# jmatta1/MCMCpp

Hardware: AMD Instinct MI355X
Metric: walker-steps/sec + acceptance rate, 16384 walkers x 32 dims, 1/2/4/8 GPU (higher is better)
Workload: dtype f64

## Files before the change

### mcmcpp_amd/csrc/mcmcpp_hip.hip

```cpp
#include <hip/hip_runtime.h>

#include <chrono>
#include <cmath>
#include <cstdarg>
#include <cstdio>
#include <cstdlib>
#include <cstring>
#include <map>
#include <mutex>
#include <new>
#include <string>
#include <thread>
#include <vector>

#include "../../include/mcmcpp_hip.h"
#define MCMCPP_DEFINE_REDUCE_KERNEL
#include "launch_table.hpp"
#include "sampler_host.hpp"
#include "split_exchange.hpp"

using namespace mcmcpp;

namespace
{
thread_local std::string g_create_error;

void parallel_memcpy(char* dst, const char* src, size_t bytes)
{
    const size_t kMinPiece = 512u << 10;
    int pieces = (int)(bytes / kMinPiece);
    if (pieces > 4) pieces = 4;
    if (pieces < 2)
    {
        std::memcpy(dst, src, bytes);
        return;
    }
    const size_t piece = ((bytes / (size_t)pieces) + 63) & ~(size_t)63;
    std::thread helpers[3];
    for (int k = 1; k < pieces; ++k)
    {
        const size_t off = piece * (size_t)k;
        const size_t len = (k == pieces - 1) ? bytes - off : piece;
        helpers[k - 1] = std::thread([=]() { std::memcpy(dst + off, src + off, len); });
    }
    std::memcpy(dst, src, piece);
    for (int k = 1; k < pieces; ++k) helpers[k - 1].join();
}

struct RegisteredCalc
{
    const void* f64;
    const void* f32;
    int params_len;
};
std::mutex g_registry_mutex;
std::map<int, RegisteredCalc> g_registry;

bool registered_calc(int calc_id, RegisteredCalc* out)
{
    std::lock_guard<std::mutex> lock(g_registry_mutex);
    std::map<int, RegisteredCalc>::const_iterator it = g_registry.find(calc_id);
    if (it == g_registry.end()) return false;
    if (out) *out = it->second;
    return true;
}

template <class T>
const LaunchTable<T>* table_for(int calc_id);
template <>
const LaunchTable<double>* table_for<double>(int calc_id)
{
    switch (calc_id)
    {
    case MCMCPP_HIP_CALC_ISO_GAUSSIAN: return launch_table_f64_iso();
    case MCMCPP_HIP_CALC_DENSE_GAUSSIAN: return launch_table_f64_dense();
    case MCMCPP_HIP_CALC_ROSENBROCK: return launch_table_f64_rosenbrock();
    case MCMCPP_HIP_CALC_SKEWED_GAUSSIAN_2D: return launch_table_f64_skewed();
    default:
    {
        RegisteredCalc r;
// ... 47 lines not shown
}
void launch_accepted_reduce(const uint32_t* partials, int partial_slots, int partial_waves, int count,
                            const StepCtl* ctl_after, const RunInfo* run, hipStream_t stream, int chains)
{
    hipLaunchKernelGGL(accepted_reduce_kernel, dim3((unsigned)count, (unsigned)(chains > 1 ? chains : 1)), dim3(256), 0, stream, partials, partial_slots,
                       partial_waves, count, ctl_after, run);
}
}

namespace
{
struct PinnedScratch
{
    alignas(64) StepCtl ctl;
    alignas(64) RunInfo run[4];
    alignas(64) StepCtl chain_ctl[kMaxChains];
    alignas(64) RunInfo chain_run[4][kMaxChains];
};
static_assert(sizeof(StepCtl) <= 64 && sizeof(RunInfo) <= 64, "a control or run record is uploaded as one 64-byte line");

int check_config(const mcmcpp_hip_config* c, std::string& err);

template <class T>
class Sampler final : public SamplerHost<T>
{
    MCMCPP_SAMPLER_HOST_NAMES;
    using Host::exchange_us_per_step, Host::xchg_bytes_per_step, Host::xchg_rollbacks, Host::xchg_cap_slots;

public:
    Sampler() {}
    ~Sampler() override
    {
        quiesce();
    }

    int init(const mcmcpp_hip_config& c)
    {
        cfg = c;
        knobs = Knobs::from_environment();
        set_shape(c);
        table = table_for<T>(c.calc_id);
        if (!table) return fail(MCMCPP_HIP_E_ARG, "calc_id %d has no kernels for this element type", c.calc_id);
        if (table->abi != kLaunchTableAbi || table->elem_size != sizeof(T))
            return fail(MCMCPP_HIP_E_ARG, "calc_id %d: the plug-in was built against other headers (table abi %08x)", c.calc_id, table->abi);

        const int lpw_log = ilog2(lpw), epl_shift = ilog2(epl / Vec16<T>::N);
        if (epl_shift >= kMaxEplShift || !table->half_step[lpw_log][epl_shift])
            return fail(MCMCPP_HIP_E_UNSUPPORTED, "no kernel for D=%d with this calculator (LPW=%d EPL=%d)", D, lpw, epl);
        calc_fn = table->calc[lpw_log][epl_shift];

        if (int rc = resolve_shard(c)) return rc;
        hipDeviceProp_t prop;
        if (int rc = open_device(c, &prop)) return rc;
        if (int rc = xchg.open(this, c)) return rc;
        K = c.num_chains > 1 ? c.num_chains : 1;
        if (K > kMaxChains) return fail(MCMCPP_HIP_E_ARG, "num_chains %d exceeds %d", K, kMaxChains);
        if (K > 1 && (shard_count != n || shard_begin != 0 || c.comm_world >= 1 || c.device_positions))
            return fail(MCMCPP_HIP_E_ARG, "num_chains > 1: whole ensembles on one device only (no shards, communicator or caller-owned positions)");
        if (int rc = open_stream(c)) return rc;

        StepShape s = {};
        s.W = W, s.D = D, s.n = n, s.lpw = lpw, s.elem_size = (int)sizeof(T), s.calc_id = c.calc_id;
        s.shard_begin = shard_begin, s.shard_count = shard_count, s.chains = K, s.comm_world = c.comm_world;
        s.num_cus = prop.multiProcessorCount;
        s.graph_steps = c.graph_steps;
        s.can_capture = own_stream || !(stream == nullptr || stream == hipStreamLegacy);
// ... 157 lines not shown
        if (!pos || !logp) return fail(MCMCPP_HIP_E_ARG, "set_state: null pointer");
        HIP_TRY(hipSetDevice(device));
        HIP_TRY(hipMemcpyAsync(d_pos, pos, sizeof(T) * (size_t)W * D * K, hipMemcpyHostToDevice, stream));
        for (int k = 0; k < K; ++k)
        {
            HIP_TRY(hipMemcpyAsync(logp_of(k), (const T*)logp + (size_t)k * W, sizeof(T) * (size_t)W, hipMemcpyHostToDevice, stream));
            HIP_TRY(hipMemsetAsync(nacc_of(k), 0, sizeof(uint32_t) * (size_t)W, stream));
        }
        HIP_TRY(hipMemsetAsync(d_diag, 0, sizeof(Diag), stream));
        half_steps = 0;
        steps_since_reset = 0;
        records_valid = false;
        int rc = write_ctl(half_steps, 0);
        if (rc) return rc;
        HIP_TRY(hipStreamSynchronize(stream));
        have_state = true;
        return MCMCPP_HIP_OK;
    }

    int run_mover(int64_t n_saved, int32_t interval, void* chain_out, uint32_t* accepted_per_step, bool to_device) override
    {
        return xchg.active() ? run_split(n_saved, interval, chain_out, accepted_per_step) : run_whole(n_saved, interval, chain_out, accepted_per_step, to_device);
    }
    int run_chains() const override { return K; }
    RunFacts run_facts() const override
    {
        RunFacts f = {};
        f.mover = Mover::Stretch;
        f.communicator = xchg.active();
        f.sharded = shard_count != n;
        f.half_done = (half_steps & 1) != 0;
        return f;
    }
    void state_abandoned() override { records_valid = false; }

    int begin_run(size_t acc_entries, const RunInfo* split_record)
    {
        if (acc_entries) HIP_TRY(hipMemsetAsync(d_acc, 0, sizeof(uint32_t) * acc_entries, stream));
        run_touched = true;
        if (int rc = write_ctl(half_steps, 0)) return rc;
        records_valid = false;
        run_info_idle = false;
        if (split_record) HIP_TRY(hipMemcpyAsync(d_run, split_record, sizeof(RunInfo), hipMemcpyHostToDevice, stream));
        if (full_fn)
        {
            for (int k = 0; k < K; ++k)
                hipLaunchKernelGGL(mark_rows_moved_kernel, dim3((unsigned)((W + 255) / 256)), dim3(256), 0, stream, nacc_of(k), W, kRowMovedBit);
            HIP_TRY(hipGetLastError());
        }
        enq_step = half_steps >> 1;
        run_step = 0;
        args_red = make_args(0);
        args_blk = make_args(1);
        return MCMCPP_HIP_OK;
    }

    using TimePoint = std::chrono::steady_clock::time_point;
    int finish_run(int64_t total, double gpu_ms, bool records_left, uint32_t* accepted_per_step, TimePoint tp1, TimePoint tp2)
    {
        last_ms = gpu_ms;
        last_launches = full_fn ? total : 2 * total;
        half_steps += 2 * (uint64_t)total;
        steps_since_reset += (uint64_t)total;
        records_valid = records_left;
        records_step = half_steps >> 1;
        records_partner2 = full_fn != nullptr;
        if (accepted_per_step) HIP_TRY(hipMemcpy(accepted_per_step, d_acc, sizeof(uint32_t) * (size_t)total * K, hipMemcpyDeviceToHost));
        host_enqueue_ms = std::chrono::duration<double, std::milli>(tp2 - tp1).count();
        return MCMCPP_HIP_OK;
    }

    int hand_out_staged(char* chain_out, const ChainPlan& cp, size_t step_bytes, StoredRange staged, int buf)
    {
        if (staged.to == staged.from) return MCMCPP_HIP_OK;
        HIP_TRY(hipEventSynchronize(ev_copied[buf]));
        for (int k = 0; k < K; ++k)
        {
            const SubchunkCopy c = subchunk_copy(step_bytes, cp.sub_saved, cp.n_saved, staged.from, staged.to - staged.from, k);
            std::memcpy(chain_out + c.dst, (const char*)h_stage[buf] + c.src, c.bytes);
        }
        publish_stored(staged.to);
        return MCMCPP_HIP_OK;
    }

    int run_whole(int64_t n_saved, int32_t interval, void* chain_out, uint32_t* accepted_per_step, bool to_device)
    {
        const int64_t total = n_saved * (int64_t)interval;

        const size_t step_bytes = sizeof(T) * (size_t)W * D;
        const ChainRequest want = {step_bytes, K, n_saved, interval, chain_out != nullptr, accepted_per_step != nullptr, full_fn != nullptr,
                                   chain_subchunk_bytes, plan.graph_steps, knobs.trickle, knobs.pinned_direct, to_device};
        void* direct_stage = pinned_question_matters(want) ? device_view_of_pinned(chain_out, step_bytes * (size_t)n_saved * K) : nullptr;
        const ChainPlan cp = plan_chain(want, direct_stage != nullptr);
        int rc = ensure_run_buffers(cp.acc_entries, cp.half_bytes, cp.ring_bytes, cp.need_host_ring);
        if (rc) return rc;
        if ((rc = begin_run(cp.acc_entries, nullptr))) return rc;
        if ((rc = ensure_graphs())) return rc;

        const TimePoint tp1 = std::chrono::steady_clock::now();
        double launch_ms = 0.0;
        if (cp.mode == ChainMode::Trickle)
            rc = run_trickle(n_saved, interval, (char*)chain_out, accepted_per_step != nullptr, step_bytes, cp, &launch_ms, (char*)direct_stage);
        else if (cp.mode == ChainMode::Device)
            rc = run_into_device_chain(n_saved, interval, (char*)chain_out, accepted_per_step != nullptr, step_bytes, cp, &launch_ms);
        StoredRange pending = {0, 0};
        int pending_buf = 0;
        for (int64_t c = 0; c < cp.n_sub && rc == MCMCPP_HIP_OK; ++c)
        {
            const int buf = (int)(c & 1);
            const StoredRange sub = cp.subchunk(c);
            for (int k = 0; k < K; ++k)
            {
                RunInfo* ri = K > 1 ? &h_pinned->chain_run[c % 4][k] : &h_pinned->run[c % 4];
                *ri = run_info_of_run(chain_out ? (char*)d_chain[buf].get() + subchunk_chain_offset(step_bytes, cp.sub_saved, k) : nullptr,
                                      accepted_per_step ? d_acc + (size_t)k * (size_t)total : nullptr, interval, step_bytes);
                ri->chain_slot_base = -sub.from;
                HIP_TRY(hipMemcpyAsync(run_of(k), ri, sizeof(RunInfo), hipMemcpyHostToDevice, stream));
            }
            HIP_TRY(hipEventRecord(ev_t0[c & 3], stream));
            rc = enqueue_steps((sub.to - sub.from) * interval);
            if (rc) break;
            HIP_TRY(hipEventRecord(ev_t1[c & 3], stream));
            if (c >= 3)
            {
                float ms = 0.f;
                HIP_TRY(hipEventSynchronize(ev_t1[(c - 3) & 3]));
                HIP_TRY(hipEventElapsedTime(&ms, ev_t0[(c - 3) & 3], ev_t1[(c - 3) & 3]));
                launch_ms += ms;
            }
            if (chain_out)
            {
                HIP_TRY(hipMemcpyAsync(h_stage[buf], d_chain[buf], subchunk_half_used(step_bytes, cp.sub_saved, sub.to - sub.from, K), hipMemcpyDeviceToHost, stream));
                HIP_TRY(hipEventRecord(ev_copied[buf], stream));
                if ((rc = hand_out_staged((char*)chain_out, cp, step_bytes, pending, pending_buf))) return rc;
                pending = sub;
// ... 172 lines not shown
    int enqueue_chunk(ChunkWindow& win, int64_t now)
    {
        const int e = win.event_slot(win.next_chunk);
        HIP_TRY(hipEventRecord(ev_t0[e], stream));
        if (const int rc = enqueue_steps(now)) return rc;
        HIP_TRY(hipEventRecord(ev_t1[e], stream));
        win.enqueued(now);
        return MCMCPP_HIP_OK;
    }
    int wait_for_oldest_chunk(const ChunkWindow& win, double* launch_ms)
    {
        const int e = win.event_slot(win.oldest);
        float ms = 0.f;
        HIP_TRY(hipEventSynchronize(ev_t1[e]));
        HIP_TRY(hipEventElapsedTime(&ms, ev_t0[e], ev_t1[e]));
        *launch_ms += ms;
        return MCMCPP_HIP_OK;
    }

    int run_trickle(int64_t n_saved, int32_t interval, char* chain_out, bool want_accepted, size_t step_bytes, const ChainPlan& cp, double* launch_ms,
                    char* direct_stage)
    {
        const int64_t total = n_saved * (int64_t)interval;
        const size_t ring_bytes = step_bytes * (size_t)cp.ring, out_bytes = step_bytes * (size_t)n_saved;
        for (int k = 0; k < K; ++k)
        {
            RunInfo* ri = &h_pinned->chain_run[0][k];
            *ri = run_info_of_run((char*)d_ring + ring_bytes * (size_t)k, want_accepted ? d_acc + (size_t)k * (size_t)total : nullptr, interval, step_bytes);
            ri->stage = cp.direct ? (void*)(direct_stage + out_bytes * (size_t)k) : (void*)((char*)h_ring + ring_bytes * (size_t)k);
            ri->slot_mask = cp.ring - 1;
            ri->slice_bytes = cp.slice_bytes;
            HIP_TRY(hipMemcpyAsync(run_of(k), ri, sizeof(RunInfo), hipMemcpyHostToDevice, stream));
        }

        TrickleWindow win(n_saved, interval, cp);
        auto copy_out = [&](StoredRange r, bool quick) {
            if (cp.direct) return;
            for (int64_t s = r.from; s < r.to; ++s)
                for (int k = 0; k < K; ++k)
                {
                    char* dst = chain_out + out_bytes * (size_t)k + step_bytes * (size_t)s;
                    const char* src = (char*)h_ring + ring_bytes * (size_t)k + step_bytes * (size_t)win.ring_slot(s);
                    if (quick)
                        parallel_memcpy(dst, src, step_bytes);
                    else
                        std::memcpy(dst, src, step_bytes);
                }
        };
        auto process_oldest = [&]() -> int {
            if (const int rc = wait_for_oldest_chunk(win, launch_ms)) return rc;
            copy_out(win.process_oldest(), win.all_enqueued());
            publish_stored(win.copied);
            return MCMCPP_HIP_OK;
        };
        while (!win.all_enqueued())
        {
            const int64_t now = win.next_length();
            while (win.must_process_oldest_before(now))
            {
                const int rc = process_oldest();
                if (rc) return rc;
            }
            if (const int rc = enqueue_chunk(win, now)) return rc;
        }
        for (int k = 0; k < K; ++k)
        {
            const size_t off = ring_bytes * (size_t)k + step_bytes * (size_t)win.ring_slot(n_saved - 1);
            char* dst = cp.direct ? chain_out + out_bytes * (size_t)k + step_bytes * (size_t)(n_saved - 1) : (char*)h_ring + off;
            HIP_TRY(hipMemcpyAsync(dst, (char*)d_ring + off, step_bytes, hipMemcpyDeviceToHost, stream));
        }
        while (win.in_flight())
        {
            const int rc = process_oldest();
            if (rc) return rc;
        }
        HIP_TRY(hipStreamSynchronize(stream));
        copy_out(win.tail(), true);
        publish_stored(win.copied);
        return MCMCPP_HIP_OK;
    }

    int run_into_device_chain(int64_t n_saved, int32_t interval, char* device_chain, bool want_accepted, size_t step_bytes, const ChainPlan& cp, double* launch_ms)
    {
        const int64_t total = n_saved * (int64_t)interval;
        for (int k = 0; k < K; ++k)
        {
            RunInfo* ri = &h_pinned->chain_run[0][k];
            *ri = run_info_of_run(device_chain + device_chain_offset(step_bytes, n_saved, k), want_accepted ? d_acc + (size_t)k * (size_t)total : nullptr, interval, step_bytes);
            HIP_TRY(hipMemcpyAsync(run_of(k), ri, sizeof(RunInfo), hipMemcpyHostToDevice, stream));
        }
        DeviceWindow win(n_saved, interval, cp);
        auto process_oldest = [&]() -> int {
            if (const int rc = wait_for_oldest_chunk(win, launch_ms)) return rc;
            publish_stored(win.process_oldest().to);
            return MCMCPP_HIP_OK;
        };
        while (!win.all_enqueued())
        {
            while (win.must_process_oldest_first())
                if (const int rc = process_oldest()) return rc;
            const int64_t now = win.next_length();
            if (const int rc = enqueue_chunk(win, now)) return rc;
        }
        while (win.in_flight())
            if (const int rc = process_oldest()) return rc;
        return MCMCPP_HIP_OK;
    }

    void* device_view_of_pinned(void* p, size_t bytes)
    {
        hipPointerAttribute_t at;
        if (hipPointerGetAttributes(&at, p) != hipSuccess || at.type != hipMemoryTypeHost || at.devicePointer == nullptr)
// ... 105 lines not shown
        if (!p.pad.empty()) HIP_TRY(hipMemcpyAsync(row + prm_row, p.pad.data(), sizeof(T) * p.pad.size(), hipMemcpyHostToDevice, stream));
        HIP_TRY(hipStreamSynchronize(stream));
        return MCMCPP_HIP_OK;
    }

    int calc_logp_chain(int32_t chain, const void* pos, int64_t count, void* out) override
    {
        if (int rc = chain_params_supported("calc_logp_chain")) return rc;
        if (chain < 0 || chain >= K) return fail(MCMCPP_HIP_E_ARG, "calc_logp_chain: chain %d outside 0..%d", chain, K - 1);
        const T* prm = d_chain_params ? d_chain_params + (size_t)chain_params_stride * (size_t)chain : d_params;
        return kernel_calc_logp(calc_fn, prm, pos, count, out);
    }

    int calc_logp_device(int32_t chain, const void* pos, int64_t count, void* out) override
    {
        if (chain < 0 || chain >= K) return fail(MCMCPP_HIP_E_ARG, "calc_logp_device: chain %d outside 0..%d", chain, K - 1);
        const T* prm = d_chain_params ? d_chain_params + (size_t)chain_params_stride * (size_t)chain : d_params;
        return kernel_calc_logp_device(calc_fn, prm, pos, count, out);
    }

    int half_step_async(int32_t color, int64_t save_slot) override
    {
        if (K > 1) return fail(MCMCPP_HIP_E_UNSUPPORTED, "half_step_async: not with several chains per handle");
        if (!have_state) return fail(MCMCPP_HIP_E_STATE, "half_step_async: set_state has not been called");
        if (color != (int)(half_steps & 1)) return fail(MCMCPP_HIP_E_ARG, "half_step_async: colour %d out of order", color);
        if (save_slot >= 0 && (!bound_chain || save_slot >= bound_slots))
            return fail(MCMCPP_HIP_E_ARG, "half_step_async: save_slot outside the bound device chain");
        HIP_TRY(hipSetDevice(device));
        if (!run_info_idle)
        {
            const int rc = upload_idle_run_info();
            if (rc) return rc;
        }
        HalfStepArgs<T> a = make_args(color, (int)((half_steps >> 1) & 1));
        a.use_ctl_save = 0;
        a.partials = nullptr;
        a.direct_save_slot = save_slot;
        half_fn(a, plan.grid_blocks_for(shard_count), stream);
        HIP_TRY(hipGetLastError());
        half_steps += 1;
        if (color == 1) steps_since_reset += 1;
        records_valid = color == 1 && shard_count == n;
        records_step = half_steps >> 1;
        records_partner2 = false;
        return MCMCPP_HIP_OK;
    }

    int bind_device_chain(void* chain, int64_t slots) override
    {
        HIP_TRY(hipSetDevice(device));
        HIP_TRY(hipStreamSynchronize(stream));
        bound_chain = chain;
        bound_slots = chain ? slots : 0;
        return upload_idle_run_info();
    }

    int shard_span(int32_t color, int64_t* off, int64_t* cnt) override
    {
        if (color != 0 && color != 1) return fail(MCMCPP_HIP_E_ARG, "shard_span: colour must be 0 or 1");
        if (off) *off = ((int64_t)(color ? n : 0) + shard_begin) * D;
        if (cnt) *cnt = (int64_t)shard_count * D;
        return MCMCPP_HIP_OK;
    }

private:
    int chain_params_supported(const char* what)
// ... 54 lines not shown
        a.n_accept = d_nacc;
        a.ctl_in = d_ctl + color;
        a.ctl_out = d_ctl + (1 - color);
        a.run = d_run;
        a.diag = d_diag;
        a.jump_lo = d_jump_lo;
        a.jump_hi = d_jump_hi;
        a.task_jump = d_task_jump;
        a.calc_params = d_params;
        a.draws = d_draws;
        a.color = color;
        a.shard_begin = shard_begin;
        a.shard_count = shard_count;
        a.passes = plan.passes;
        a.partials = d_partials;
        a.partial_slots = plan.partial_slots;
        a.partial_waves = plan.partial_waves;
        a.draw_parity = 0;
        a.pos_alt = d_pos_alt;
        a.logp_alt = d_logp + W;
        a.pos_parity = 0;
        a.calc_params_padded = d_params_padded;
        a.chains = K;
        a.params_chain_stride = chain_params_stride;
        a.draw_wave = plan.half_draw_wave;
        return a;
    }

    U128 engine_state_before(uint64_t h, int k = 0) const
    {
        return apply(pcg_jump(inc, (unsigned __int128)3 * (unsigned)n * (unsigned __int128)h), state0_of[k]);
    }

    int write_ctl(uint64_t at, uint64_t step_in_run, int32_t interval = 1)
    {
        const bool refill = !(records_valid && records_step == (at >> 1) && (!full_fn || records_partner2));
        for (int k = 0; k < K; ++k)
        {
            StepCtl* c = K > 1 ? &h_pinned->chain_ctl[k] : &h_pinned->ctl;
            c->state = engine_state_before(at, k);
            const U128 state1 = apply(half_jump, c->state);
            c->state2 = apply(half_jump, state1);
            c->half_step = at;
            c->step_in_run = step_in_run;
            c->chain_slot = (long long)(step_in_run / (uint64_t)interval);
            c->save_phase = (uint32_t)(step_in_run % (uint64_t)interval);
            c->partial_slot = (uint32_t)(step_in_run % (uint64_t)plan.partial_slots);
            HIP_TRY(hipMemcpyAsync(ctl_of(k) + (at & 1), c, sizeof(StepCtl), hipMemcpyHostToDevice, stream));
            if (refill)
            {
                const int parity = (int)((at >> 1) & 1);
                HalfStepArgs<T> fr = make_args(0, parity), fb = make_args(1, parity);
                fr.draws = fb.draws = d_draws + draws_chain_offset(k, n);
                launch_fill_draws(fr, c->state, nullptr, stream);
                launch_fill_draws(fb, state1, full_fn ? &c->state : nullptr, stream);
                HIP_TRY(hipGetLastError());
            }
        }
        if (refill)
        {
            records_valid = true;
            records_step = at >> 1;
            records_partner2 = full_fn != nullptr;
        }
        HIP_TRY(hipStreamSynchronize(stream));
        return MCMCPP_HIP_OK;
    }

    void enqueue_step(int parity, int pos_parity, int batch_slot = -1)
    {
        if (full_fn)
        {
            HalfStepArgs<T>& a = args_red;
            a.draw_parity = parity;
            a.pos_parity = pos_parity;
            a.ctl_in = d_ctl + pos_parity;
            a.ctl_out = d_ctl + (1 - pos_parity);
            a.draw_wave = plan.full_draw_wave;
            if (batch_slot >= 0)
            {
                a.draw_wave = 2;
                a.draw_parity = 0;
                a.draws = d_draws_batch + (size_t)batch_slot * 2 * (size_t)n;
            }
            full_fn(a, plan.full_grid_blocks_for(a.shard_count), stream);
            a.draws = d_draws;
            return;
        }
        args_red.draw_parity = parity;
        args_blk.draw_parity = parity;
        half_fn(args_red, plan.grid_blocks_for(args_red.shard_count), stream);
        half_fn(args_blk, plan.grid_blocks_for(args_blk.shard_count), stream);
    }

    void fill_batch(int pos_parity, int count)
    {
        HalfStepArgs<T> a = args_red;
        a.draws = d_draws;
// ... 88 lines not shown
        if (half_bytes > 0 && ev_copied[0] == nullptr)
        {
            for (int k = 0; k < 2; ++k) HIP_TRY(hipEventCreateWithFlags(ev_copied[k].replace(), hipEventDisableTiming));
        }
        for (int k = 0; k < 2; ++k)
        {
            if (grow(d_chain[k], half_bytes, stream)) return fail(MCMCPP_HIP_E_NOMEM, "run: cannot allocate %zu bytes of device chain", half_bytes);
            if (grow(h_stage[k], half_bytes, stream)) return fail(MCMCPP_HIP_E_NOMEM, "run: cannot allocate %zu bytes of pinned staging", half_bytes);
        }
        return MCMCPP_HIP_OK;
    }

    mcmcpp_hip_config cfg;
    Knobs knobs;
    const LaunchTable<T>* table = nullptr;
    StepPlan plan;
    typename LaunchTable<T>::HalfStepFn half_fn = nullptr;
    typename LaunchTable<T>::HalfStepFn full_fn = nullptr;
    T* d_pos_alt = nullptr;
    uint64_t run_step = 0;
    typename LaunchTable<T>::CalcFn calc_fn = nullptr;
    int shard_begin = 0, shard_count = 0;
    size_t chain_subchunk_bytes = 0;
    Event ev_copied[2];
    DeviceBuffer<char> arena;
    size_t arena_used = 0;
    DeviceBuffer<char> d_ring;
    PinnedBuffer<char> h_ring;
    DeviceBuffer<T> d_chain[2];
    PinnedBuffer<char> h_stage[2];
    DeviceBuffer<uint32_t> d_acc;
    bool own_pos = false;
    Event ev_t0[4], ev_t1[4];
    T *d_params = nullptr, *d_params_padded = nullptr;
    DeviceBuffer<T> d_chain_params;
    int chain_params_stride = 0;
    StepCtl* d_ctl = nullptr;
    RunInfo* d_run = nullptr;
    DrawRec<T>* d_draws = nullptr;
    DeviceBuffer<DrawRec<T>> d_draws_batch;
    DeviceBuffer<Affine128> d_step_jump;
    uint32_t* d_partials = nullptr;
    Affine128 *d_jump_lo = nullptr, *d_jump_hi = nullptr, *d_task_jump = nullptr;
    bool records_valid = false, records_partner2 = false, run_info_idle = false;
    uint64_t records_step = 0;
    PinnedBuffer<PinnedScratch> h_pinned;
    U128 inc;
    U128 state0_of[kMaxChains];
    int K = 1;
    Affine128 half_jump;
    HalfStepArgs<T> args_red, args_blk;
    std::vector<GraphExec> graph_cache;
    uint64_t half_steps = 0, enq_step = 0;
    void* bound_chain = nullptr;
    int64_t bound_slots = 0;
    SplitExchange<T> xchg;
};

int check_config(const mcmcpp_hip_config* c, std::string& err)
{
    char buf[256];
#define BAD(...)                              \
    do                                        \
    {                                         \
        snprintf(buf, sizeof buf, __VA_ARGS__); \
        err = buf;                            \
// ... 342 lines not shown
```

### mcmcpp_amd/csrc/run_plan.hpp

```cpp
#pragma once

#include <cstddef>
#include <cstdint>

namespace mcmcpp
{
inline int64_t stored_steps_per_subchunk(size_t budget, size_t stored_step_bytes, int64_t n_saved)
{
    int64_t s = (int64_t)(budget / stored_step_bytes);
    const int64_t eighth = (n_saved + 7) / 8;
    if (s > eighth) s = eighth;
    if (s < 1) s = 1;
    return s;
}

enum class ChainMode { Nothing, Subchunks, Trickle, Device };

struct ChainRequest
{
    size_t step_bytes;
    int chains;
    int64_t n_saved;
    int32_t interval;
    bool chain_out, want_accepted;
// ... 80 lines not shown
    int64_t total() const { return n_saved * interval; }
    bool all_enqueued() const { return enq == total(); }
    bool in_flight() const { return next_chunk > oldest; }
    static int event_slot(int64_t chunk) { return (int)(chunk & 3); }
    void enqueued(int64_t now)
    {
        enq += now;
        chunk_end[event_slot(next_chunk)] = enq;
        ++next_chunk;
    }
};

struct DeviceWindow : ChunkWindow
{
    int64_t announced = 0;

    DeviceWindow(int64_t n_saved_, int64_t interval_, const ChainPlan& p) : ChunkWindow(n_saved_, interval_, p.chunk_steps) {}

    int64_t next_length() const { return total() - enq < chunk_steps ? total() - enq : chunk_steps; }
    bool must_process_oldest_first() const { return next_chunk - oldest >= 2; }
    StoredRange process_oldest()
    {
        const StoredRange r = {announced, chunk_end[event_slot(oldest)] / interval};
        announced = r.to;
        ++oldest;
        return r;
    }
};

struct TrickleWindow : ChunkWindow
{
    int64_t ring;
    bool direct;
    int64_t copied = 0;

    TrickleWindow(int64_t n_saved_, int64_t interval_, const ChainPlan& p) : ChunkWindow(n_saved_, interval_, p.chunk_steps), ring(p.ring), direct(p.direct) {}

    int64_t ring_slot(int64_t stored_step) const { return stored_step & (ring - 1); }

    int64_t next_length() const
    {
        int64_t now = (total() - enq < chunk_steps) ? total() - enq : chunk_steps;
        if (!direct && now == total() - enq && now > interval) now -= interval;
        return now;
    }
    bool must_process_oldest_before(int64_t now) const
    {
        return in_flight() && (next_chunk - oldest >= 2 || (!direct && enq + now > (copied + ring + 1) * interval));
    }
    StoredRange process_oldest()
    {
        const int64_t complete = chunk_end[event_slot(oldest)] / interval - 1;
        const StoredRange r = {copied, complete > copied ? complete : copied};
        copied = r.to;
        ++oldest;
        return r;
    }
    StoredRange tail()
    {
        const StoredRange r = {copied, n_saved};
        copied = n_saved;
        return r;
    }
};

inline size_t subchunk_chain_offset(size_t step_bytes, int64_t sub_saved, int k) { return step_bytes * (size_t)sub_saved * (size_t)k; }
struct SubchunkCopy { size_t dst, src, bytes; };
inline SubchunkCopy subchunk_copy(size_t step_bytes, int64_t sub_saved, int64_t n_saved, int64_t first, int64_t count, int k)
{
    return {step_bytes * ((size_t)n_saved * (size_t)k + (size_t)first), subchunk_chain_offset(step_bytes, sub_saved, k), step_bytes * (size_t)count};
}
inline size_t subchunk_half_used(size_t step_bytes, int64_t sub_saved, int64_t now, int chains)
{
    return step_bytes * (size_t)sub_saved * (size_t)(chains - 1) + step_bytes * (size_t)now;
}

struct PiecePlan
{
    int64_t n_saved;
    int64_t piece_saved, n_pieces;
    size_t chain_bytes, acc_entries;

    StoredRange piece(int64_t c) const
    {
        const int64_t first = c * piece_saved;
        return {first, n_saved - first < piece_saved ? n_saved : first + piece_saved};
    }
};
inline PiecePlan pieces_of(int64_t n_saved, int64_t piece_saved)
{
    PiecePlan p = {};
    p.n_saved = n_saved;
    p.piece_saved = piece_saved;
    p.n_pieces = n_saved > 0 ? (n_saved + piece_saved - 1) / piece_saved : 0;
    return p;
}

// ... 162 lines not shown
```

### mcmcpp_amd/csrc/step_plan.hpp

```cpp
#pragma once

#include <cstddef>
#include <cstdlib>
#include <optional>

#include "../../include/mcmcpp_hip.h"

namespace mcmcpp
{
constexpr int kWavesPerBlock = 4;
constexpr size_t kJumpEntryBytes = 32;

inline int pow2_at_least(int v)
{
    int p = 1;
    while (p < v) p <<= 1;
    return p;
}
inline int ilog2(int v)
{
    int l = 0;
    while ((1 << l) < v) ++l;
    return l;
}
// ... 5 lines not shown
    return {lpw, n2 / lpw, (D % base == 0) ? 1 : 0};
}

inline std::optional<long> env_long(const char* name)
{
    const char* v = std::getenv(name);
    if (v && *v) return std::strtol(v, nullptr, 10);
    return std::nullopt;
}
inline long env_long(const char* name, long fallback) { return env_long(name).value_or(fallback); }

struct Knobs
{
    long passes;
    long waves_per_simd;
    long matrix_core_min_walkers;
    std::optional<long> matrix_core_4pass;
    long matrix_core_late;
    long full_step;
    long full_step_max_walkers;
    long task_table_mb;
    long chain_subchunk_mb;
    long graph_steps;
    long trickle;
    long no_draw_wave;
    long batch_draws;
    long pinned_direct;
    long comm_full_step;
    long comm_compact;
    long comm_compact_cap;
    long comm_compact_chunk;
    std::optional<long> de_scan_run;
    std::optional<long> de_batch;
    static Knobs from_environment()
    {
        Knobs k;
        k.passes = env_long("MCMCPP_HIP_PASSES", 0);
        k.waves_per_simd = env_long("MCMCPP_HIP_WAVES_PER_SIMD", 2);
        k.matrix_core_min_walkers = env_long("MCMCPP_HIP_MATRIX_CORE_MIN_WALKERS", 0);
        k.matrix_core_4pass = env_long("MCMCPP_HIP_MATRIX_CORE_4PASS_WALKERS");
        k.matrix_core_late = env_long("MCMCPP_HIP_MATRIX_CORE_LATE_DRAWS", 49152);
        k.full_step = env_long("MCMCPP_HIP_FULL_STEP", 1);
        k.full_step_max_walkers = env_long("MCMCPP_HIP_FULL_STEP_MAX_WALKERS", -1);
        k.task_table_mb = env_long("MCMCPP_HIP_TASK_TABLE_MB", 16);
        k.chain_subchunk_mb = env_long("MCMCPP_HIP_CHAIN_SUBCHUNK_MB", 32);
        k.graph_steps = env_long("MCMCPP_HIP_GRAPH_STEPS", -1);
        k.trickle = env_long("MCMCPP_HIP_TRICKLE", 1);
        k.no_draw_wave = env_long("MCMCPP_HIP_NO_DRAW_WAVE", 0);
        k.batch_draws = env_long("MCMCPP_HIP_BATCH_DRAWS", -1);
        k.pinned_direct = env_long("MCMCPP_HIP_PINNED_DIRECT", 1);
        k.comm_full_step = env_long("MCMCPP_HIP_COMM_FULL_STEP", 1);
        k.comm_compact = env_long("MCMCPP_HIP_COMM_COMPACT", 1);
        k.comm_compact_cap = env_long("MCMCPP_HIP_COMM_COMPACT_CAP", 0);
        k.comm_compact_chunk = env_long("MCMCPP_HIP_COMM_COMPACT_CHUNK", 256);
        if (k.comm_compact_chunk < 1) k.comm_compact_chunk = 1;
        k.de_scan_run = env_long("MCMCPP_HIP_DE_SCAN_RUN");
        k.de_batch = env_long("MCMCPP_HIP_DE_BATCH");
        return k;
    }
};

struct StepShape
{
    int W, D, n;
    int lpw;
    int elem_size;
    int calc_id;
    int shard_begin, shard_count;
    int chains;
    int comm_world;
    int num_cus;
    int graph_steps;
    bool can_capture;
    bool half_step_mc[3], full_step, full_step_mc, de_update_mc;
};

enum class HalfStepKernel { Plain, MatrixCore8, MatrixCore16, MatrixCore16Late };
enum class FullStepKernel { None, Plain, MatrixCore };

struct StepPlan
{
    HalfStepKernel half = HalfStepKernel::Plain;
    FullStepKernel full = FullStepKernel::None;
    int passes = 1;
    int step_lpw = 1;
    int full_wpb = 1;
    int graph_steps = 32;
    int batch_draws = 0;
    int partial_slots = 1, partial_waves = 0;
    bool have_task_table = false;
// ... 85 lines not shown
```

Measured before the change: 2.856 billion.

## Move trickle chain copy-out to background threads and skip run-start stream sync

Adds a CopyOut worker pool that performs the host-side memcpy from the pinned ring into the user chain buffer asynchronously. The ring-reuse rule now waits on copier progress rather than copying inline. The final-step tail is split into pieces with per-piece events so host copies can start while later pieces are still transferring. begin_run no longer blocks on a stream synchronize for the control upload; it records an event that is waited on lazily. This aims to overlap host copies with GPU work and remove synchronous stalls, at the cost of threading complexity and extra bookkeeping for cancellation and ordering.

```diff
diff --git a/mcmcpp_amd/csrc/copy_out.hpp b/mcmcpp_amd/csrc/copy_out.hpp
--- /dev/null
+++ b/mcmcpp_amd/csrc/copy_out.hpp
@@ -0,0 +1,155 @@
+#pragma once
+
+#include <atomic>
+#include <chrono>
+#include <condition_variable>
+#include <cstddef>
+#include <cstdint>
+#include <cstring>
+#include <functional>
+#include <mutex>
+#include <thread>
+
+namespace mcmcpp
+{
+struct CopyJob
+{
+    char* dst;
+    const char* src;
+    size_t bytes;
+    int64_t stored_step;
+    bool tail;
+};
+
+class CopyOut
+{
+public:
+    static constexpr int kQueue = 64;
+    static constexpr int kMaxHelpers = 2;
+
+    explicit CopyOut(int helpers = 0, long delay_us = 0, std::function<void(int64_t)> on_stored = nullptr)
+        : helpers_(helpers < 0 ? 0 : (helpers > kMaxHelpers ? kMaxHelpers : helpers)), delay_us_(delay_us > 0 ? delay_us : 0), on_stored_(std::move(on_stored))
+    {
+        try
+        {
+            worker_ = std::thread([this]() { work(false); });
+            for (int k = 0; k < helpers_; ++k) helper_[k] = std::thread([this]() { work(true); });
+        }
+        catch (...)
+        {
+            stop_and_join();
+            throw;
+        }
+    }
+    CopyOut(const CopyOut&) = delete;
+    CopyOut& operator=(const CopyOut&) = delete;
+    ~CopyOut()
+    {
+        cancel();
+        stop_and_join();
+    }
+
+    int threads() const { return 1 + helpers_; }
+
+    void begin_run()
+    {
+        drain();
+        copied_.store(0, std::memory_order_release);
+    }
+
+    void push(const CopyJob& job)
+    {
+        std::unique_lock<std::mutex> lock(m_);
+        quiet_cv_.wait(lock, [this]() { return pushed_ - retired_ < (uint64_t)kQueue; });
+        slot_[pushed_ % kQueue].job = job;
+        slot_[pushed_ % kQueue].done = false;
+        ++pushed_;
+        lock.unlock();
+        work_cv_.notify_all();
+    }
+
+    int64_t copied() const { return copied_.load(std::memory_order_acquire); }
+
+    int64_t wait_copied(int64_t count)
+    {
+        std::unique_lock<std::mutex> lock(m_);
+        quiet_cv_.wait(lock, [&]() { return copied() >= count || retired_ == pushed_; });
+        return copied();
+    }
+
+    void drain()
+    {
+        std::unique_lock<std::mutex> lock(m_);
+        quiet_cv_.wait(lock, [this]() { return retired_ == pushed_; });
+    }
+
+    void cancel()
+    {
+        std::unique_lock<std::mutex> lock(m_);
+        pushed_ = taken_;
+        quiet_cv_.wait(lock, [this]() { return retired_ == pushed_; });
+    }
+
+private:
+    void stop_and_join()
+    {
+        {
+            std::lock_guard<std::mutex> lock(m_);
+            stop_ = true;
+        }
+        work_cv_.notify_all();
+        if (worker_.joinable()) worker_.join();
+        for (int k = 0; k < kMaxHelpers; ++k)
+            if (helper_[k].joinable()) helper_[k].join();
+    }
+
+    struct Slot
+    {
+        CopyJob job;
+        bool done;
+    };
+
+    void work(bool helper)
+    {
+        std::unique_lock<std::mutex> lock(m_);
+        for (;;)
+        {
+            work_cv_.wait(lock, [&]() { return stop_ || (taken_ < pushed_ && (!helper || slot_[taken_ % kQueue].job.tail)); });
+            if (stop_) return;
+            const uint64_t mine = taken_++;
+            const CopyJob job = slot_[mine % kQueue].job;
+            const bool more = taken_ < pushed_;
+            lock.unlock();
+            if (more) work_cv_.notify_all();
+            if (delay_us_ > 0) std::this_thread::sleep_for(std::chrono::microseconds(delay_us_));
+            std::memcpy(job.dst, job.src, job.bytes);
+            lock.lock();
+            slot_[mine % kQueue].done = true;
+            int64_t reached = 0;
+            while (retired_ < taken_ && slot_[retired_ % kQueue].done)
+            {
+                const int64_t s = slot_[retired_ % kQueue].job.stored_step;
+                if (s > reached) reached = s;
+                ++retired_;
+            }
+            const bool moved = reached > copied();
+            if (moved) copied_.store(reached, std::memory_order_release);
+            lock.unlock();
+            if (moved && on_stored_) on_stored_(reached);
+            quiet_cv_.notify_all();
+            lock.lock();
+        }
+    }
+
+    const int helpers_;
+    const long delay_us_;
+    const std::function<void(int64_t)> on_stored_;
+    std::mutex m_;
+    std::condition_variable work_cv_, quiet_cv_;
+    Slot slot_[kQueue];
+    uint64_t pushed_ = 0, taken_ = 0, retired_ = 0;
+    bool stop_ = false;
+    std::atomic<int64_t> copied_{0};
+    std::thread worker_, helper_[kMaxHelpers];
+};
+}
diff --git a/mcmcpp_amd/csrc/mcmcpp_hip.hip b/mcmcpp_amd/csrc/mcmcpp_hip.hip
--- a/mcmcpp_amd/csrc/mcmcpp_hip.hip
+++ b/mcmcpp_amd/csrc/mcmcpp_hip.hip
@@ -7,14 +7,15 @@
 #include <cstdlib>
 #include <cstring>
 #include <map>
+#include <memory>
 #include <mutex>
 #include <new>
 #include <string>
-#include <thread>
 #include <vector>
 
 #include "../../include/mcmcpp_hip.h"
 #define MCMCPP_DEFINE_REDUCE_KERNEL
+#include "copy_out.hpp"
 #include "launch_table.hpp"
 #include "sampler_host.hpp"
 #include "split_exchange.hpp"
@@ -24,28 +25,6 @@
 namespace
 {
 thread_local std::string g_create_error;
-
-void parallel_memcpy(char* dst, const char* src, size_t bytes)
-{
-    const size_t kMinPiece = 512u << 10;
-    int pieces = (int)(bytes / kMinPiece);
-    if (pieces > 4) pieces = 4;
-    if (pieces < 2)
-    {
-        std::memcpy(dst, src, bytes);
-        return;
-    }
-    const size_t piece = ((bytes / (size_t)pieces) + 63) & ~(size_t)63;
-    std::thread helpers[3];
-    for (int k = 1; k < pieces; ++k)
-    {
-        const size_t off = piece * (size_t)k;
-        const size_t len = (k == pieces - 1) ? bytes - off : piece;
-        helpers[k - 1] = std::thread([=]() { std::memcpy(dst + off, src + off, len); });
-    }
-    std::memcpy(dst, src, piece);
-    for (int k = 1; k < pieces; ++k) helpers[k - 1].join();
-}
 
 struct RegisteredCalc
 {
@@ -159,6 +138,7 @@
     ~Sampler() override
     {
         quiesce();
+        copier.reset();
     }
 
     int init(const mcmcpp_hip_config& c)
@@ -382,13 +362,17 @@
         f.half_done = (half_steps & 1) != 0;
         return f;
     }
-    void state_abandoned() override { records_valid = false; }
+    void state_abandoned() override
+    {
+        records_valid = false;
+        if (copier) copier->cancel();
+    }
 
     int begin_run(size_t acc_entries, const RunInfo* split_record)
     {
         if (acc_entries) HIP_TRY(hipMemsetAsync(d_acc, 0, sizeof(uint32_t) * acc_entries, stream));
         run_touched = true;
-        if (int rc = write_ctl(half_steps, 0)) return rc;
+        if (int rc = write_ctl(half_steps, 0, 1, plan.batch_draws == 0, split_record != nullptr)) return rc;
         records_valid = false;
         run_info_idle = false;
         if (split_record) HIP_TRY(hipMemcpyAsync(d_run, split_record, sizeof(RunInfo), hipMemcpyHostToDevice, stream));
@@ -450,7 +434,10 @@
         const TimePoint tp1 = std::chrono::steady_clock::now();
         double launch_ms = 0.0;
         if (cp.mode == ChainMode::Trickle)
+        {
             rc = run_trickle(n_saved, interval, (char*)chain_out, accepted_per_step != nullptr, step_bytes, cp, &launch_ms, (char*)direct_stage);
+            if (rc != MCMCPP_HIP_OK && copier) copier->cancel();
+        }
         else if (cp.mode == ChainMode::Device)
             rc = run_into_device_chain(n_saved, interval, (char*)chain_out, accepted_per_step != nullptr, step_bytes, cp, &launch_ms);
         StoredRange pending = {0, 0};
@@ -689,52 +676,120 @@
             ri->slice_bytes = cp.slice_bytes;
             HIP_TRY(hipMemcpyAsync(run_of(k), ri, sizeof(RunInfo), hipMemcpyHostToDevice, stream));
         }
+        if (!cp.direct)
+        {
+            if (int rc = ensure_copier()) return rc;
+            copier->begin_run();
+        }
 
         TrickleWindow win(n_saved, interval, cp);
-        auto copy_out = [&](StoredRange r, bool quick) {
-            if (cp.direct) return;
+        auto hand = [&](StoredRange r, bool tail) {
             for (int64_t s = r.from; s < r.to; ++s)
                 for (int k = 0; k < K; ++k)
-                {
-                    char* dst = chain_out + out_bytes * (size_t)k + step_bytes * (size_t)s;
-                    const char* src = (char*)h_ring + ring_bytes * (size_t)k + step_bytes * (size_t)win.ring_slot(s);
-                    if (quick)
-                        parallel_memcpy(dst, src, step_bytes);
-                    else
-                        std::memcpy(dst, src, step_bytes);
-                }
+                    push_copy(chain_out + out_bytes * (size_t)k + step_bytes * (size_t)s, (char*)h_ring + ring_bytes * (size_t)k + step_bytes * (size_t)win.ring_slot(s),
+                              step_bytes, k == K - 1 ? s + 1 : 0, tail);
         };
         auto process_oldest = [&]() -> int {
             if (const int rc = wait_for_oldest_chunk(win, launch_ms)) return rc;
-            copy_out(win.process_oldest(), win.all_enqueued());
-            publish_stored(win.copied);
+            if (cp.direct)
+                publish_stored(win.process_oldest().to);
+            else
+                hand(win.hand_oldest(), win.all_enqueued());
             return MCMCPP_HIP_OK;
         };
         while (!win.all_enqueued())
         {
             const int64_t now = win.next_length();
-            while (win.must_process_oldest_before(now))
-            {
-                const int rc = process_oldest();
-                if (rc) return rc;
+            for (;;)
+            {
+                if (!cp.direct) win.copied_up_to(copier->copied());
+                if (win.must_process_oldest_before(now))
+                {
+                    if (const int rc = process_oldest()) return rc;
+                }
+                else if (win.must_wait_for_copies_before(now))
+                    copier->wait_copied(win.copies_needed_before(now));
+                else
+                    break;
             }
             if (const int rc = enqueue_chunk(win, now)) return rc;
         }
+        for (;;)
+        {
+            if (!cp.direct) win.copied_up_to(copier->copied());
+            if (win.must_process_oldest_before_tail())
+            {
+                if (const int rc = process_oldest()) return rc;
+            }
+            else if (win.must_wait_for_copies_before_tail())
+                copier->wait_copied(win.copies_needed_before_tail());
+            else
+                break;
+        }
+        const int pieces = cp.direct ? 1 : tail_pieces(step_bytes);
+        if (!cp.direct)
+            while (ev_piece.size() < (size_t)pieces * (size_t)K)
+            {
+                ev_piece.emplace_back();
+                HIP_TRY(hipEventCreateWithFlags(ev_piece.back().replace(), hipEventDisableTiming));
+            }
         for (int k = 0; k < K; ++k)
-        {
-            const size_t off = ring_bytes * (size_t)k + step_bytes * (size_t)win.ring_slot(n_saved - 1);
-            char* dst = cp.direct ? chain_out + out_bytes * (size_t)k + step_bytes * (size_t)(n_saved - 1) : (char*)h_ring + off;
-            HIP_TRY(hipMemcpyAsync(dst, (char*)d_ring + off, step_bytes, hipMemcpyDeviceToHost, stream));
-        }
+            for (int p = 0; p < pieces; ++p)
+            {
+                const TailPiece tp = tail_piece(step_bytes, pieces, p);
+                const size_t off = ring_bytes * (size_t)k + step_bytes * (size_t)win.ring_slot(n_saved - 1) + tp.off;
+                char* dst = cp.direct ? chain_out + out_bytes * (size_t)k + step_bytes * (size_t)(n_saved - 1) + tp.off : (char*)h_ring + off;
+                HIP_TRY(hipMemcpyAsync(dst, (char*)d_ring + off, tp.bytes, hipMemcpyDeviceToHost, stream));
+                if (!cp.direct) HIP_TRY(hipEventRecord(ev_piece[(size_t)k * pieces + p], stream));
+            }
         while (win.in_flight())
         {
             const int rc = process_oldest();
             if (rc) return rc;
         }
+        if (cp.direct)
+        {
+            HIP_TRY(hipStreamSynchronize(stream));
+            publish_stored(win.tail().to);
+            return MCMCPP_HIP_OK;
+        }
+        win.hand_tail();
+        for (int k = 0; k < K; ++k)
+            for (int p = 0; p < pieces; ++p)
+            {
+                const TailPiece tp = tail_piece(step_bytes, pieces, p);
+                const size_t off = ring_bytes * (size_t)k + step_bytes * (size_t)win.ring_slot(n_saved - 1) + tp.off;
+                HIP_TRY(hipEventSynchronize(ev_piece[(size_t)k * pieces + p]));
+                copier->push({chain_out + out_bytes * (size_t)k + step_bytes * (size_t)(n_saved - 1) + tp.off, (char*)h_ring + off, tp.bytes,
+                              k == K - 1 && p == pieces - 1 ? n_saved : 0, true});
+            }
+        copier->drain();
+        win.copied_up_to(copier->copied());
         HIP_TRY(hipStreamSynchronize(stream));
-        copy_out(win.tail(), true);
-        publish_stored(win.copied);
-        return MCMCPP_HIP_OK;
+        return MCMCPP_HIP_OK;
+    }
+
+    int ensure_copier()
+    {
+        if (copier) return MCMCPP_HIP_OK;
+        try
+        {
+            copier = std::make_unique<CopyOut>(CopyOut::kMaxHelpers, knobs.test_copy_delay_us, [this](int64_t count) { publish_stored(count); });
+        }
+        catch (const std::exception& e)
+        {
+            return fail(MCMCPP_HIP_E_NOMEM, "run: cannot start the copy threads: %s", e.what());
+        }
+        return MCMCPP_HIP_OK;
+    }
+    void push_copy(char* dst, const char* src, size_t bytes, int64_t stored_after, bool tail)
+    {
+        const size_t piece = tail ? kTailPieceBytes : bytes;
+        for (size_t off = 0; off < bytes; off += piece)
+        {
+            const size_t len = bytes - off < piece ? bytes - off : piece;
+            copier->push({dst + off, src + off, len, off + len == bytes ? stored_after : 0, tail});
+        }
     }
 
     int run_into_device_chain(int64_t n_saved, int32_t interval, char* device_chain, bool want_accepted, size_t step_bytes, const ChainPlan& cp, double* launch_ms)
@@ -906,6 +961,8 @@
             const int rc = upload_idle_run_info();
             if (rc) return rc;
         }
+        if (color == 0 && !records_valid && plan.batch_draws > 0)
+            if (int rc = write_ctl(half_steps, 0)) return rc;
         HalfStepArgs<T> a = make_args(color, (int)((half_steps >> 1) & 1));
         a.use_ctl_save = 0;
         a.partials = nullptr;
@@ -1026,9 +1083,15 @@
         return apply(pcg_jump(inc, (unsigned __int128)3 * (unsigned)n * (unsigned __int128)h), state0_of[k]);
     }
 
-    int write_ctl(uint64_t at, uint64_t step_in_run, int32_t interval = 1)
-    {
-        const bool refill = !(records_valid && records_step == (at >> 1) && (!full_fn || records_partner2));
+    int write_ctl(uint64_t at, uint64_t step_in_run, int32_t interval = 1, bool prime = true, bool wait = true)
+    {
+        if (ctl_upload_pending)
+        {
+            HIP_TRY(hipEventSynchronize(ev_ctl));
+            ctl_upload_pending = false;
+        }
+        const bool refill = prime && !(records_valid && records_step == (at >> 1) && (!full_fn || records_partner2));
+        if (!prime) records_valid = false;
         for (int k = 0; k < K; ++k)
         {
             StepCtl* c = K > 1 ? &h_pinned->chain_ctl[k] : &h_pinned->ctl;
@@ -1057,7 +1120,14 @@
             records_step = at >> 1;
             records_partner2 = full_fn != nullptr;
         }
-        HIP_TRY(hipStreamSynchronize(stream));
+        if (wait)
+            HIP_TRY(hipStreamSynchronize(stream));
+        else
+        {
+            if (ev_ctl == nullptr) HIP_TRY(hipEventCreateWithFlags(ev_ctl.replace(), hipEventDisableTiming));
+            HIP_TRY(hipEventRecord(ev_ctl, stream));
+            ctl_upload_pending = true;
+        }
         return MCMCPP_HIP_OK;
     }
 
@@ -1212,6 +1282,10 @@
     DeviceBuffer<uint32_t> d_acc;
     bool own_pos = false;
     Event ev_t0[4], ev_t1[4];
+    Event ev_ctl;
+    bool ctl_upload_pending = false;
+    std::vector<Event> ev_piece;
+    std::unique_ptr<CopyOut> copier;
     T *d_params = nullptr, *d_params_padded = nullptr;
     DeviceBuffer<T> d_chain_params;
     int chain_params_stride = 0;
diff --git a/mcmcpp_amd/csrc/run_plan.hpp b/mcmcpp_amd/csrc/run_plan.hpp
--- a/mcmcpp_amd/csrc/run_plan.hpp
+++ b/mcmcpp_amd/csrc/run_plan.hpp
@@ -136,6 +136,7 @@
 {
     int64_t ring;
     bool direct;
+    int64_t handed = 0;
     int64_t copied = 0;
 
     TrickleWindow(int64_t n_saved_, int64_t interval_, const ChainPlan& p) : ChunkWindow(n_saved_, interval_, p.chunk_steps), ring(p.ring), direct(p.direct) {}
@@ -148,25 +149,63 @@
         if (!direct && now == total() - enq && now > interval) now -= interval;
         return now;
     }
-    bool must_process_oldest_before(int64_t now) const
-    {
-        return in_flight() && (next_chunk - oldest >= 2 || (!direct && enq + now > (copied + ring + 1) * interval));
-    }
-    StoredRange process_oldest()
+    bool ring_rule_blocks(int64_t now) const { return !direct && enq + now > (copied + ring + 1) * interval; }
+    bool must_process_oldest_before(int64_t now) const { return in_flight() && (next_chunk - oldest >= 2 || (ring_rule_blocks(now) && copied == handed)); }
+    bool must_wait_for_copies_before(int64_t now) const { return ring_rule_blocks(now) && copied < handed; }
+    int64_t copies_needed_before(int64_t now) const
+    {
+        const int64_t need = (enq + now + interval - 1) / interval - ring - 1;
+        return need < handed ? need : handed;
+    }
+    int64_t copies_needed_before_tail() const { return direct || n_saved < ring ? 0 : n_saved - ring; }
+    bool must_process_oldest_before_tail() const { return in_flight() && handed < copies_needed_before_tail(); }
+    bool must_wait_for_copies_before_tail() const { return copied < copies_needed_before_tail() && copied < handed; }
+    void copied_up_to(int64_t count)
+    {
+        if (count > copied) copied = count < handed ? count : handed;
+    }
+    StoredRange hand_oldest()
     {
         const int64_t complete = chunk_end[event_slot(oldest)] / interval - 1;
-        const StoredRange r = {copied, complete > copied ? complete : copied};
-        copied = r.to;
+        const StoredRange r = {handed, complete > handed ? complete : handed};
+        handed = r.to;
         ++oldest;
         return r;
     }
+    StoredRange process_oldest()
+    {
+        const StoredRange r = hand_oldest();
+        copied = handed;
+        return r;
+    }
+    StoredRange hand_tail()
+    {
+        const StoredRange r = {handed, n_saved};
+        handed = n_saved;
+        return r;
+    }
     StoredRange tail()
     {
-        const StoredRange r = {copied, n_saved};
-        copied = n_saved;
+        const StoredRange r = hand_tail();
+        copied = handed;
         return r;
     }
 };
+
+constexpr size_t kTailPieceBytes = (size_t)1 << 20;
+constexpr int kTailMaxPieces = 8;
+struct TailPiece { size_t off, bytes; };
+inline int tail_pieces(size_t step_bytes)
+{
+    const size_t n = (step_bytes + kTailPieceBytes - 1) / kTailPieceBytes;
+    return n < 1 ? 1 : (n > (size_t)kTailMaxPieces ? kTailMaxPieces : (int)n);
+}
+inline TailPiece tail_piece(size_t step_bytes, int pieces, int p)
+{
+    const size_t each = ((step_bytes + (size_t)pieces - 1) / (size_t)pieces + 63) & ~(size_t)63;
+    const size_t off = each * (size_t)p < step_bytes ? each * (size_t)p : step_bytes;
+    return {off, p == pieces - 1 || step_bytes - off < each ? step_bytes - off : each};
+}
 
 inline size_t subchunk_chain_offset(size_t step_bytes, int64_t sub_saved, int k) { return step_bytes * (size_t)sub_saved * (size_t)k; }
 struct SubchunkCopy { size_t dst, src, bytes; };
diff --git a/mcmcpp_amd/csrc/step_plan.hpp b/mcmcpp_amd/csrc/step_plan.hpp
--- a/mcmcpp_amd/csrc/step_plan.hpp
+++ b/mcmcpp_amd/csrc/step_plan.hpp
@@ -61,6 +61,7 @@
     long comm_compact_chunk;
     std::optional<long> de_scan_run;
     std::optional<long> de_batch;
+    long test_copy_delay_us;
     static Knobs from_environment()
     {
         Knobs k;
@@ -85,6 +86,7 @@
         if (k.comm_compact_chunk < 1) k.comm_compact_chunk = 1;
         k.de_scan_run = env_long("MCMCPP_HIP_DE_SCAN_RUN");
         k.de_batch = env_long("MCMCPP_HIP_DE_BATCH");
+        k.test_copy_delay_us = env_long("MCMCPP_HIP_TEST_COPY_DELAY_US", 0);
         return k;
     }
 };
```

New measurement: 2.880 billion, median of 6. About the same (+0.8%).
